# bjg-gh/style_transfer_visualizer

Hardware: AMD Instinct MI355X
Metric: optimization steps/sec at 512² and 1024², 1/2/4/8 MI355X (higher is better)
Workload: dtype bf16; 1 GPU; single 512x512 image per GPU, L-BFGS (max_iter=1, history 100), VGG19 bf16 storage / fp32 accumulate, fp32 Gram, --no-video (BASELINE.json configs[1]); weights: synthetic He-scaled; size=512, images=1, init_method=random, parallelism=replicas x1 (independent images), lbfgs_history_prefill_steps=95, world_size=1

## Files before the change

include/stv.h:

```cpp
#ifndef STV_H_
#define STV_H_

#include <stddef.h>
#include <stdint.h>

#ifdef __cplusplus
extern "C" {
#endif

enum { STV_F32 = 0, STV_BF16 = 1, STV_BF16X3 = 2 };

enum {
  STV_OK = 0,
  STV_ERR_ARG = 1,
  STV_ERR_LAUNCH = 2,
  STV_ERR_ALLOC = 3,
  STV_ERR_GRAPH = 4
};

enum {
  STV_RELU_IN = 1,
  STV_RELU_OUT = 2,
  STV_MASK = 4,
  STV_ACCUM = 8,
// ... 140 lines not shown
#define STV_GIF_THREADS 256
#define STV_GIF_MAX_BLOCKS 2048
#define STV_GIF_HIST_BINS 32768
int stv_frame_hist(const uint8_t* frame_hwc, size_t n_pixels, uint32_t* hist, void* stream);
int stv_gif_map(const uint8_t* frame_hwc, uint8_t* index_hw, int H, int W, const uint8_t* palette, int n_colors, int spread,
                void* stream);

#define STV_JPEG_DCT_TABLE                                        \
  {{2896, 2896, 2896, 2896, 2896, 2896, 2896, 2896},              \
   {4017, 3406, 2276, 799, -799, -2276, -3406, -4017},            \
   {3784, 1567, -1567, -3784, -3784, -1567, 1567, 3784},          \
   {3406, -799, -4017, -2276, 2276, 4017, 799, -3406},            \
   {2896, -2896, -2896, 2896, 2896, -2896, -2896, 2896},          \
   {2276, -4017, 799, 3406, -3406, -799, 4017, -2276},            \
   {1567, -3784, 3784, -1567, -1567, 3784, -3784, 1567},          \
   {799, -2276, 3406, -4017, 4017, -3406, 2276, -799}}
#define STV_JPEG_DCT_THREADS 256
#define STV_JPEG_THREADS 256
#define STV_JPEG_MAX_BLOCK_BITS 1664
#define STV_JPEG_MAX_DIM 65535
int stv_jpeg_dct(const uint8_t* frame_hwc, const int* qtabs, int H, int W, int16_t* coef, void* stream);
int stv_jpeg_block_bits(const int16_t* coef, int n_frames, int blocks_per_frame, uint32_t* bits, void* stream);
int stv_jpeg_scan(const uint32_t* bits, int n_frames, int blocks_per_frame, uint32_t* offsets, uint32_t* totals, void* stream);
int stv_jpeg_emit(const int16_t* coef, const uint32_t* offsets, const uint32_t* base, int n_frames, int blocks_per_frame,
                  uint8_t* stream_bytes, size_t capacity, void* stream);

int stv_loss_combine(const float* parts, const int32_t* table, const float* scale,
                     int n_terms, float style_w, float content_w, float* losses,
                     float* scores, void* stream);
int stv_loss_combine_log(const float* parts, const int32_t* table, const float* scale,
                         int n_terms, float style_w, float content_w, float* losses,
                         float* scores, float* log_ring, int log_capacity, uint32_t* log_count,
                         uint32_t* log_seq, void* stream);
int stv_host_mailbox_alloc(size_t bytes, void** out);
void stv_host_mailbox_free(void* p);


typedef struct stv_lbfgs_state stv_lbfgs_state;
size_t stv_lbfgs_state_bytes(int history);
size_t stv_lbfgs_workspace_bytes(size_t n, int history);
int stv_lbfgs_step(float* x, const float* grad, void* state, void* workspace, size_t n,
                   int history, int m_max, float lr, float tol_grad, float tol_change,
                   void* stream);
size_t stv_lbfgsc_state_bytes(int history);
size_t stv_lbfgsc_workspace_bytes(size_t n, int history);
int stv_lbfgsc_step(float* x, const float* grad, void* state, void* workspace, size_t n,
                    int history, int m_max, float lr, float tol_grad, float tol_change,
                    void* stream);
int stv_lbfgsc_dots(const float* grad, void* state, void* workspace, size_t n, int history, int m_max, void* stream);
int stv_lbfgsc_apply(float* x, const float* grad, void* state, void* workspace, size_t n, int history, float lr,
                     float tol_grad, float tol_change, void* stream);
size_t stv_lbfgsc_dots_offset(size_t n, int history, int* count, int* max_index);
int stv_lbfgsc_geometry(size_t n, int history, size_t* nn, int* tile_a, int* ntiles, int* pgroups, int* tile_b);
int stv_lbfgsc_iter(float* x, const float* grad, const float* loss, void* state, void* workspace, size_t n,
                    int history, int m_max, int iters_per_step, float lr, float tol_grad, float tol_change,
                    void* stream);
int stv_lbfgsc_iter_reset(void* state, void* stream);
int stv_adam_step(float* x, const float* grad, float* exp_avg, float* exp_avg_sq, size_t n,
                  float lr, float one_minus_beta1, float beta2, float one_minus_beta2, float eps,
                  float bias_c1, float bias_c2_sqrt, void* stream);

enum {
  STV_OP_CONV_FIRST_FWD = 1, STV_OP_CONV_FIRST_DGRAD, STV_OP_CONV, STV_OP_POOL_FWD,
  STV_OP_POOL_BWD, STV_OP_RELU_FWD, STV_OP_RELU_BWD, STV_OP_GRAM_PARTIAL,
  STV_OP_GRAM_FINISH, STV_OP_CONTENT_LOSS, STV_OP_CONTENT_GRAD, STV_OP_LOSS_COMBINE,
  STV_OP_MEMSET, STV_OP_GRAM_MULTI, STV_OP_LBFGS_STEP, STV_OP_LBFGS_ITER, STV_OP_TV,
  STV_OP_LAP, STV_OP_MASK_SPLIT, STV_OP_AVGPOOL_FWD, STV_OP_AVGPOOL_BWD
};
typedef struct {
  int32_t op, dtype, flags, taps;
  int32_t H, W, cin, cout;
  int64_t n;
  float f0, f1, f2, f3;
  const void* p0; const void* p1; const void* p2; const void* p3;
  void* q0; void* q1; void* q2; void* q3;
} stv_op_t;

typedef struct stv_program stv_program;
int stv_program_create(const stv_op_t* ops, int n_ops, stv_program** out);
int stv_program_run(stv_program* prog, int use_graph, void* stream);
int stv_program_profile(stv_program* prog, void* stream, float* ms_out, int n_out);
int stv_program_profile_reps(stv_program* prog, void* stream, int reps, float* ms_out, int n_out);
int stv_program_op_count(const stv_program* prog);
void stv_program_destroy(stv_program* prog);

#ifdef __cplusplus
}
#endif
#endif
```

style_transfer_visualizer_amd/_lib.py:

```python
from __future__ import annotations

import ctypes
import os
from ctypes import c_float, c_int, c_int32, c_int64, c_size_t, c_void_p

_HERE = os.path.dirname(os.path.abspath(__file__))
LIB_PATH = os.environ.get("STV_LIB_PATH") or os.path.join(_HERE, "libstv_hip.so")

STV_F32, STV_BF16, STV_BF16X3 = 0, 1, 2
TUNE_BF16X3 = 6
RELU_IN, RELU_OUT, MASK, ACCUM, W_BLOCKED, POOL_IDX, POOL_ROUTE, POOL_ONLY = 1, 2, 4, 8, 16, 32, 64, 128

(OP_CONV_FIRST_FWD, OP_CONV_FIRST_DGRAD, OP_CONV, OP_POOL_FWD, OP_POOL_BWD, OP_RELU_FWD,
 OP_RELU_BWD, OP_GRAM_PARTIAL, OP_GRAM_FINISH, OP_CONTENT_LOSS, OP_CONTENT_GRAD,
 OP_LOSS_COMBINE, OP_MEMSET, OP_GRAM_MULTI, OP_LBFGS_STEP, OP_LBFGS_ITER, OP_TV, OP_LAP, OP_MASK_SPLIT, OP_AVGPOOL_FWD, OP_AVGPOOL_BWD) = range(1, 22)

CONTENT_LOSS_PARTS = 256
TV_LOSS_PARTS = 256
TV_THREADS, TV_VEC = 1024, 4
KIND_STYLE, KIND_CONTENT, KIND_EXTRA = 0, 1, 2
LAP_POOL, LAP_LOSS, LAP_GRAD = 0, 1, 2
LAP_POOLS = (1, 2, 4, 8, 16, 32)
LAP_THREADS, LAP_TILE_H, LAP_TILE_W, LAP_LOSS_PARTS, LAP_GRAD_MAX_BLOCKS, LAP_VEC = 256, 8, 32, 256, 512, 4
MASK_MAX_REGIONS, MASK_SPLIT_THREADS, MASK_SPLIT_MAX_BLOCKS = 4, 256, 1024
# ... 70 lines not shown
    "stv_conv_tune": (c_int, [c_int, c_int, c_int, c_int, c_int, c_int, c_void_p]),
    "stv_conv_tune_export": (c_int, [ctypes.POINTER(c_int), c_int]),
    "stv_conv_tune_import": (c_int, [ctypes.POINTER(c_int), c_int]),
    "stv_conv_next_weights": (None, [c_void_p, c_size_t]),
    "stv_conv_num_configs": (c_int, []),
    "stv_conv_last_launch": (c_int, []),
    "stv_conv_uses_ws": (c_int, [c_int, c_int, c_int, c_int, c_int, c_int, c_int, c_int, c_int]),
    "stv_conv_config": (c_int, [c_int, c_int, c_int, c_int, c_int, c_int]),
    "stv_maxpool_fwd": (c_int, [c_void_p, c_void_p, c_int, c_int, c_int, c_int, c_void_p]),
    "stv_maxpool_bwd": (c_int, [c_void_p, c_void_p, c_void_p, c_int, c_int, c_int, c_int, c_int, c_void_p]),
    "stv_avgpool_fwd": (c_int, [c_void_p, c_void_p, c_int, c_int, c_int, c_int, c_int, c_void_p]),
    "stv_avgpool_bwd": (c_int, [c_void_p, c_void_p, c_void_p, c_int, c_int, c_int, c_int, c_int, c_void_p]),
    "stv_relu_fwd": (c_int, [c_void_p, c_void_p, c_size_t, c_int, c_void_p]),
    "stv_relu_bwd": (c_int, [c_void_p, c_void_p, c_void_p, c_size_t, c_int, c_int, c_void_p]),
    "stv_gram_partial": (c_int, [c_void_p, c_void_p, c_int, c_int, c_int, c_void_p]),
    "stv_gram_finish": (c_int, [c_void_p, c_void_p, c_void_p, c_void_p, c_void_p, c_int, c_int, c_float, c_float, c_float, c_void_p, c_int, c_void_p]),
    "stv_gram_multi": (c_int, [c_void_p, c_int, c_int, c_void_p]),
    "stv_content_loss": (c_int, [c_void_p, c_void_p, c_void_p, c_size_t, c_int, c_void_p]),
    "stv_content_loss_grad": (c_int, [c_void_p, c_void_p, c_void_p, c_void_p, c_size_t, c_float, c_int, c_void_p]),
    "stv_content_grad": (c_int, [c_void_p, c_void_p, c_void_p, c_size_t, c_float, c_void_p, c_int, c_int, c_void_p]),
    "stv_tv": (c_int, [c_void_p, c_void_p, c_void_p, c_int, c_int, c_int, c_float, c_int, c_void_p]),
    "stv_lap": (c_int, [c_void_p, c_void_p, c_void_p, c_void_p, c_void_p, c_int, c_int, c_int, c_int, c_float, c_int, c_int, c_void_p]),
    "stv_mask_split": (c_int, [c_void_p, c_void_p, c_void_p, c_size_t, c_int, c_int, c_int, c_void_p]),
    "stv_resize2x": (c_int, [c_void_p, c_void_p, c_int, c_int, c_int, c_int, c_void_p]),
    "stv_resize_axis": (c_int, [c_void_p, c_void_p, c_int, c_int, c_int, c_int, c_int, c_void_p, c_void_p, c_void_p, c_int, c_void_p]),
    "stv_color_stats": (c_int, [c_void_p, c_void_p, c_int, c_int, c_void_p]),
    "stv_color_affine": (c_int, [c_void_p, c_void_p, ctypes.POINTER(c_float), c_int, c_int, c_void_p]),
    "stv_luma_transfer": (c_int, [c_void_p, c_void_p, c_void_p, c_int, c_int, ctypes.POINTER(c_float), ctypes.POINTER(c_float), c_void_p]),
    "stv_kmeans_assign": (c_int, [c_void_p, c_void_p, c_void_p, c_void_p, c_int, c_int, c_int, c_void_p]),
    "stv_gram_blend": (c_int, [c_void_p, c_void_p, ctypes.POINTER(c_float), c_int, c_int64, c_void_p]),
    "stv_image_to_u8": (c_int, [c_void_p, c_void_p, c_int, c_int, ctypes.POINTER(c_float), ctypes.POINTER(c_float), c_int, c_void_p]),
    "stv_frame_hist": (c_int, [c_void_p, c_size_t, c_void_p, c_void_p]),
    "stv_gif_map": (c_int, [c_void_p, c_void_p, c_int, c_int, c_void_p, c_int, c_int, c_void_p]),
    "stv_jpeg_dct": (c_int, [c_void_p, ctypes.POINTER(c_int), c_int, c_int, c_void_p, c_void_p]),
    "stv_jpeg_block_bits": (c_int, [c_void_p, c_int, c_int, c_void_p, c_void_p]),
    "stv_jpeg_scan": (c_int, [c_void_p, c_int, c_int, c_void_p, c_void_p, c_void_p]),
    "stv_jpeg_emit": (c_int, [c_void_p, c_void_p, c_void_p, c_int, c_int, c_void_p, c_size_t, c_void_p]),
    "stv_loss_combine": (c_int, [c_void_p, c_void_p, c_void_p, c_int, c_float, c_float, c_void_p, c_void_p, c_void_p]),
    "stv_loss_combine_log": (c_int, [c_void_p, c_void_p, c_void_p, c_int, c_float, c_float, c_void_p, c_void_p, c_void_p,
                                     c_int, c_void_p, c_void_p, c_void_p]),
    "stv_host_mailbox_alloc": (c_int, [c_size_t, ctypes.POINTER(c_void_p)]),
    "stv_host_mailbox_free": (None, [c_void_p]),
    "stv_lbfgs_state_bytes": (c_size_t, [c_int]),
    "stv_lbfgs_workspace_bytes": (c_size_t, [c_size_t, c_int]),
    "stv_lbfgs_step": (c_int, [c_void_p, c_void_p, c_void_p, c_void_p, c_size_t, c_int, c_int, c_float, c_float, c_float, c_void_p]),
    "stv_lbfgsc_state_bytes": (c_size_t, [c_int]),
    "stv_lbfgsc_workspace_bytes": (c_size_t, [c_size_t, c_int]),
    "stv_lbfgsc_step": (c_int, [c_void_p, c_void_p, c_void_p, c_void_p, c_size_t, c_int, c_int, c_float, c_float, c_float, c_void_p]),
    "stv_lbfgsc_dots": (c_int, [c_void_p, c_void_p, c_void_p, c_size_t, c_int, c_int, c_void_p]),
    "stv_lbfgsc_apply": (c_int, [c_void_p, c_void_p, c_void_p, c_void_p, c_size_t, c_int, c_float, c_float, c_float, c_void_p]),
    "stv_lbfgsc_dots_offset": (c_size_t, [c_size_t, c_int, ctypes.POINTER(c_int), ctypes.POINTER(c_int)]),
    "stv_lbfgsc_geometry": (c_int, [c_size_t, c_int, ctypes.POINTER(c_size_t), ctypes.POINTER(c_int), ctypes.POINTER(c_int),
                                    ctypes.POINTER(c_int), ctypes.POINTER(c_int)]),
    "stv_lbfgsc_iter": (c_int, [c_void_p, c_void_p, c_void_p, c_void_p, c_void_p, c_size_t, c_int, c_int, c_int, c_float, c_float, c_float,
                                c_void_p]),
    "stv_lbfgsc_iter_reset": (c_int, [c_void_p, c_void_p]),
    "stv_adam_step": (c_int, [c_void_p, c_void_p, c_void_p, c_void_p, c_size_t, c_float, c_float, c_float, c_float, c_float, c_float, c_float, c_void_p]),
    "stv_program_create": (c_int, [ctypes.POINTER(StvOp), c_int, ctypes.POINTER(c_void_p)]),
    "stv_program_run": (c_int, [c_void_p, c_int, c_void_p]),
    "stv_program_profile": (c_int, [c_void_p, c_void_p, ctypes.POINTER(c_float), c_int]),
    "stv_program_profile_reps": (c_int, [c_void_p, c_void_p, c_int, ctypes.POINTER(c_float), c_int]),
    "stv_program_op_count": (c_int, [c_void_p]),
    "stv_program_destroy": (None, [c_void_p]),
}

_lib = None


def load() -> ctypes.CDLL:
    global _lib
    if _lib is not None:
        return _lib
    import torch
    if not os.path.exists(LIB_PATH):
        msg = (f"{LIB_PATH} not found: build it with `python -c 'import __graft_entry__ as g; g.build()'` "
               "(hipcc --offload-arch=gfx950). There is no CPU/eager fallback for this path.")
        raise RuntimeError(msg)
    lib = ctypes.CDLL(LIB_PATH)
    for name, (res, args) in SIGNATURES.items():
        fn = getattr(lib, name)
        fn.restype = res
        fn.argtypes = args
    _lib = lib
    _import_tile_table(lib)
    return lib


TILE_TABLE_PATH = os.environ.get("STV_TILE_TABLE") or os.path.join(_HERE, "conv_tiles_gfx950.json")
tile_table_info: dict = {"source": None, "entries": 0}


def _import_tile_table(lib: ctypes.CDLL) -> None:
    import json
    import warnings
    if not os.path.exists(TILE_TABLE_PATH):
        return

    def give_up(why: str) -> None:
        lib.stv_conv_tune_import(None, 0)
        tile_table_info.update(source=None, entries=0, ignored=f"{os.path.basename(TILE_TABLE_PATH)}: {why}")
        warnings.warn(f"conv tile table {TILE_TABLE_PATH} ignored ({why}): analytic tile choices", RuntimeWarning, stacklevel=3)
    try:
        with open(TILE_TABLE_PATH) as fh:
            doc = json.load(fh)
        rows = [int(v) for e in doc.get("entries", []) for v in (e["H"], e["W"], e["cin"], e["cout"], e["taps"], e["elem_bytes"], e["cfg"])]
    except (OSError, ValueError, KeyError, TypeError, AttributeError) as exc:
# ... 42 lines not shown
```

style_transfer_visualizer_amd/csrc/lbfgs_compact.hip:

```cpp
#include <stddef.h>
#include <stdlib.h>

#include <type_traits>

#include "stv_common.h"

namespace {

constexpr int MAX_HIST = 128;
constexpr int MAX_S = MAX_HIST + 1;
constexpr int NSCAL = 8;
constexpr int SC_DTMAX = 7;

struct CState {
  int n_iter, hist_len, head, skip, no_update, pushed, steps_seen, step_pos;
  float t, H_diag, gtd, gmax, ys, yy, cg, prev_loss;
  float ro[MAX_S];
  float cs[MAX_S];
  float cy[MAX_S];
};

struct CWs {
  float* d;
  float* prev_g;
// ... 97 lines not shown
  const int per = (m + pgroups - 1) / pgroups;
  const int j_end = (pgrp + 1) * per < m ? (pgrp + 1) * per : m;
  for (int jj = pgrp * per; jj < j_end; ++jj) {
    const int slot = (head + jj) % S;
    const float* __restrict__ sj = w.S + (size_t)slot * nn;
    const float* __restrict__ yj = w.Y + (size_t)slot * nn;
    double a0 = 0.0, a1 = 0.0, a2 = 0.0, a4 = 0.0;
#pragma unroll
    for (int u = 0; u < U; ++u) {
      const size_t idx = base + (size_t)(u * 256 + tid) * 4;
      const f32x4 s4 = ldh4(sj + idx);
      const f32x4 y4 = ldh4(yj + idx);
#pragma unroll
      for (int e = 0; e < 4; ++e) {
        const double sd = (double)s4[e], yd = (double)y4[e];
        const double gd = (double)gv[u][e], cd = (double)yv[u][e];
        a0 = fma(sd, gd, a0);
        a1 = fma(yd, gd, a1);
        a2 = fma(sd, cd, a2);
        a4 = fma(yd, cd, a4);
      }
    }
    a0 = wave_sum_d_dpp(a0); a1 = wave_sum_d_dpp(a1); a2 = wave_sum_d_dpp(a2); a4 = wave_sum_d_dpp(a4);
    if (lane == 0) {
      double* o = w.part + (size_t)(jj * 5) * nparts + p;
      o[0] = a0; o[(size_t)nparts] = a1; o[(size_t)2 * nparts] = a2; o[(size_t)3 * nparts] = 0.0;
      o[(size_t)4 * nparts] = a4;
    }
  }
  if (pgrp != 0) return;
  gmax = wave_max(gmax);
  gl1 = wave_sum_d(gl1); gg = wave_sum_d(gg); gs = wave_sum_d(gs); gy = wave_sum_d(gy); sy = wave_sum_d(sy); yy = wave_sum_d(yy);
  if (lane == 0) {
    double* o = w.partd + p;
    o[0] = (double)gmax; o[(size_t)nparts] = gl1; o[(size_t)2 * nparts] = gg; o[(size_t)3 * nparts] = gs;
    o[(size_t)4 * nparts] = gy; o[(size_t)5 * nparts] = sy; o[(size_t)6 * nparts] = yy;
  }
  if constexpr (ITER) {
    dtmax = wave_max(dtmax);
    if (lane == 0) w.partd[(size_t)SC_DTMAX * nparts + p] = (double)dtmax;
  }
}
template <int U>
__global__ __launch_bounds__(256) void pass_a_kernel(const float* __restrict__ g, const CState* st, CWs w,
                                                     size_t n, size_t nn, int hist, int nparts, int ntiles, int pgroups) {
  pass_a_body<U, false>(g, st, w, n, nn, hist, nparts, ntiles, pgroups);
}
template <int U>
__global__ __launch_bounds__(256) void pass_a_iter_kernel(const float* __restrict__ g, const CState* st, CWs w,
                                                          size_t n, size_t nn, int hist, int nparts, int ntiles, int pgroups) {
  pass_a_body<U, true>(g, st, w, n, nn, hist, nparts, ntiles, pgroups);
}

__global__ __launch_bounds__(256) void reduce_kernel(const CState* st, CWs w, int hist, int nparts) {
  __shared__ double red[256];
  const int m = st->hist_len;
  int dot = blockIdx.x;
  const bool scalar = dot >= 5 * m;
  if (scalar) dot = 5 * hist + (dot - 5 * m);
  if (dot >= 5 * hist + NSCAL) return;
  const double* __restrict__ src = w.part + (size_t)dot * nparts;
  const double* __restrict__ srcd = w.partd + (size_t)(scalar ? dot - 5 * hist : 0) * nparts;
  const bool is_max = dot == 5 * hist || dot == 5 * hist + SC_DTMAX;
  double acc = 0.0;
  for (int i = threadIdx.x; i < nparts; i += 256) {
    const double v = scalar ? srcd[i] : src[i];
    acc = is_max ? fmax(acc, v) : acc + v;
  }
  red[threadIdx.x] = acc;
  __syncthreads();
  for (int s = 128; s > 0; s >>= 1) {
    if (threadIdx.x < s)
      red[threadIdx.x] = is_max ? fmax(red[threadIdx.x], red[threadIdx.x + s]) : red[threadIdx.x] + red[threadIdx.x + s];
    __syncthreads();
  }
  if (threadIdx.x == 0) w.dots[scalar ? 5 * MAX_HIST + (dot - 5 * hist) : dot] = red[0];
}

#ifdef STV_SOLVE_STAMPS
__device__ unsigned long long g_solve_stamps[8];
#define SOLVE_STAMP(k) do { if (threadIdx.x == 0) g_solve_stamps[k] = wall_clock64(); } while (0)
#else
#define SOLVE_STAMP(k) do { } while (0)
#endif

template <bool ITER>
__device__ __forceinline__ void solve_body(CState* st, CWs w, int hist, float lr, float tol_grad, float tol_change,
                                           const float* __restrict__ loss, int iters) {
  extern __shared__ __attribute__((aligned(16))) char smem_raw[];
  const int S = hist + 1;
  const int P = hist | 1;
  double* sT = reinterpret_cast<double*>(smem_raw);
  __shared__ int sh_skip, sh_pushed, sh_m, sh_head, sh_cslot, sh_mold, sh_pos;
  __shared__ float sh_newro, sh_H;
  __shared__ double sh_gs[MAX_S], sh_gy[MAX_S], sh_ro[MAX_S];
  __shared__ double sh_bp[2][128];
  __shared__ double sh_cy[128];
  const int tid = threadIdx.x;
  const double* D = w.dots;
  const double* SC = w.dots + 5 * MAX_HIST;
  const double gmax = SC[0], gl1 = SC[1], gg = SC[2], gsc = SC[3], gyc = SC[4], ys = SC[5], yy = SC[6];
  SOLVE_STAMP(0);

  if (tid == 0) {
    struct Hdr { int n_iter, hist_len, head, skip, no_update, pushed, steps_seen, step_pos;
                 float t, H_diag, gtd, gmax, ys, yy, cg, prev_loss; };
    static_assert(sizeof(Hdr) == 64, "header layout");
    Hdr h = *reinterpret_cast<const Hdr*>(st);
    h.steps_seen += 1;
    h.gmax = (float)gmax;
    h.no_update = 0;
    h.pushed = 0;
    int skip = ((float)gmax <= tol_grad) ? 1 : 0;
    int pos = 1;
    float loss_now = 0.f;
    if constexpr (ITER) {
      loss_now = *loss;
      int done = h.step_pos < 0 ? -h.step_pos : h.step_pos;
      bool dead = h.step_pos < 0;
      if (done >= iters) { done = 0; dead = false; }
      pos = done + 1;
      if (pos > 1 && !skip)
        skip = ((float)SC[SC_DTMAX] <= tol_change || fabs((double)loss_now - (double)h.prev_loss) < (double)tol_change) ? 1 : 0;
      if (dead) skip = 1;
      h.step_pos = pos >= iters ? 0 : (skip ? -pos : pos);
    }
    h.skip = skip;
    int pushed = 0;
    const int m_old = h.hist_len;
    const int cslot = (h.head + m_old) % S;
    if (!skip) {
      h.n_iter += 1;
      if (h.n_iter == 1) {
        h.hist_len = 0;
        h.head = 0;
        h.H_diag = 1.0f;
      } else {
        h.ys = (float)ys;
        h.yy = (float)yy;
        if ((float)ys > 1e-10f) {
          pushed = 1;
          if (h.hist_len == hist) h.head = (h.head + 1) % S;
          else h.hist_len += 1;
          st->ro[cslot] = 1.0f / (float)ys;
          h.H_diag = (float)ys / (float)yy;
          sh_newro = 1.0f / (float)ys;
        }
      }
      if (h.n_iter == 1) {
// ... 26 lines not shown
      w.YY[(size_t)slot * S + cslot] = y_j_yc;
      w.YY[(size_t)cslot * S + slot] = y_j_yc;
    }
    if (tid == 0) {
      w.SY[(size_t)cslot * S + cslot] = ys;
      w.YY[(size_t)cslot * S + cslot] = yy;
    }
  }
  for (int i = tid; i < m; i += 256) {
    const int slot = (head + i) % S;
    sh_ro[i] = (sh_pushed && slot == cslot) ? (double)sh_newro : (double)st->ro[slot];
    if (sh_pushed && slot == cslot) {
      sh_gs[i] = gsc;
      sh_gy[i] = gyc;
    } else {
      const int jj = (slot - old_head + S) % S;
      sh_gs[i] = D[jj * 5 + 0];
      sh_gy[i] = D[jj * 5 + 1];
    }
  }
  __threadfence_block();
  __syncthreads();
  SOLVE_STAMP(2);
  {
    const int j = tid & 127, i0 = tid >> 7;
    if (j < m) {
      int col = head + j;
      if (col >= S) col -= S;
      constexpr int FB = 50;
      for (int ib = i0; ib < m; ib += 2 * FB) {
        double v[FB];
#pragma unroll
        for (int k = 0; k < FB; ++k) {
          int i = ib + 2 * k;
          if (i >= m) i = m - 1;
          int rs = head + i;
          if (rs >= S) rs -= S;
          const double* __restrict__ src = (i < j) ? w.SY : w.YY;
          v[k] = src[(size_t)rs * S + col];
        }
#pragma unroll
        for (int k = 0; k < FB; ++k) {
          const int i = ib + 2 * k;
          if (i < m) sT[i * P + j] = v[k];
        }
      }
    }
  }
  __syncthreads();
  SOLVE_STAMP(3);

  const int lane = tid & 63, wave4 = tid >> 6;
  const int j0 = lane, j1 = lane + 64;
  auto bcast = [](double v, int src) -> double {
    const long long bits = __double_as_longlong(v);
    const int lo = __builtin_amdgcn_readlane((int)(bits & 0xFFFFFFFFll), src);
    const int hi = __builtin_amdgcn_readlane((int)(bits >> 32), src);
    return __longlong_as_double(((long long)hi << 32) | (unsigned int)lo);
  };
  const double gs0 = j0 < m ? sh_gs[j0] : 0.0, gs1 = j1 < m ? sh_gs[j1] : 0.0;
  const double gy0 = j0 < m ? sh_gy[j0] : 0.0, gy1 = j1 < m ? sh_gy[j1] : 0.0;
  const double ro0 = j0 < m ? sh_ro[j0] : 0.0, ro1 = j1 < m ? sh_ro[j1] : 0.0;
  double cy0 = 0.0, cy1 = 0.0, cs0 = 0.0, cs1 = 0.0, al0 = 0.0, al1 = 0.0;
  double a0 = 0.0, a1 = 0.0;
  double cg = -1.0;
  constexpr int CH = 4;
  using hi_t = std::integral_constant<bool, true>;
  using lo_t = std::integral_constant<bool, false>;
  const int r0 = (j0 < m ? j0 : m - 1) * P, r1 = (j1 < m ? j1 : m - 1) * P;
  const int q0 = j0 < m ? j0 : m - 1, q1 = j1 < m ? j1 : m - 1;
  const float ro0f = (float)ro0, ro1f = (float)ro1;
  auto walk1 = [&](auto HI, int ifrom, int ito) {
    constexpr bool hi = decltype(HI)::value;
    if (ifrom < ito) return;
    double n0[CH], n1[CH];
    auto fetch = [&](int ib) {
#pragma unroll
      for (int k = 0; k < CH; ++k) {
        const int i = max(ib - k, 0);
        const double v0 = sT[r0 + i];
        if (hi) {
          n0[k] = v0;
          const double v1 = sT[r1 + i];
          n1[k] = (j1 < i) ? v1 : 0.0;
        } else {
          n0[k] = (j0 < i) ? v0 : 0.0;
        }
      }
    };
    fetch(ifrom);
    for (int ib = ifrom; ib >= ito; ib -= CH) {
      double c0[CH], c1[CH];
#pragma unroll
      for (int k = 0; k < CH; ++k) { c0[k] = n0[k]; c1[k] = hi ? n1[k] : 0.0; }
      if (ib - CH >= ito) fetch(ib - CH);
#pragma unroll
      for (int k = 0; k < CH; ++k) {
        const int i = ib - k;
        if (i < ito) break;
        const int src = hi ? i - 64 : i;
        const double cand = (double)(float)((float)(cg * (hi ? gs1 : gs0) + (hi ? a1 : a0)) * (hi ? ro1f : ro0f));
        const double al = bcast(cand, src);
        if (lane == src) {
          if (hi) { al1 = al; cy1 = -al; } else { al0 = al; cy0 = -al; }
        }
        a0 -= al * c0[k];
        if (hi) a1 -= al * c1[k];
      }
    }
  };
  if (m > 0) {
    walk1(hi_t{}, m - 1, 64);
    walk1(lo_t{}, m - 1 < 63 ? m - 1 : 63, 0);
  }
  SOLVE_STAMP(4);
  const double H = (double)sh_H;
  cg *= H; cy0 *= H; cy1 *= H;
  double b0 = cg * gy0, b1 = cg * gy1;
  {
    if (wave4 == 0) {
      sh_cy[j0] = cy0;
      sh_cy[j1] = cy1;
    }
    __syncthreads();
    const int row = tid & 127, part = tid >> 7;
    double chunk_sum[2] = {0.0, 0.0};
    if (row < m) {
      const int rb = row * P;
#pragma unroll
      for (int c = 0; c < 2; ++c) {
        const int jb = (2 * part + c) * 32;
        double acc = 0.0;
#pragma unroll
        for (int kb = 0; kb < 32; kb += 16) {
          double cv[16], tv[16];
#pragma unroll
          for (int k = 0; k < 16; ++k) {
            const int j = jb + kb + k;
            const int jc = j < m ? j : m - 1;
            cv[k] = sh_cy[j];
            tv[k] = sT[(jc <= row) ? rb + jc : jc * P + row];
          }
#pragma unroll
          for (int k = 0; k < 16; ++k) acc = fma(cv[k], tv[k], acc);
        }
        chunk_sum[c] = acc;
      }
    }
    sh_bp[part][row] = chunk_sum[0] + chunk_sum[1];
    __syncthreads();
    if (tid >= 64) return;
    b0 = b0 + (sh_bp[0][lane] + sh_bp[1][lane]);
    b1 = b1 + (sh_bp[0][64 + lane] + sh_bp[1][64 + lane]);
  }
  SOLVE_STAMP(5);
  auto walk3 = [&](auto HI, int ifrom, int ito) {
    constexpr bool hi = decltype(HI)::value;
    if (ifrom >= ito) return;
    double n0[CH], n1[CH];
    auto fetch = [&](int ib) {
#pragma unroll
      for (int k = 0; k < CH; ++k) {
        const int i = min(ib + k, m - 1);
        const double v1 = sT[i * P + q1];
        if (!hi) {
          const double v0 = sT[i * P + q0];
          n0[k] = (j0 > i) ? v0 : 0.0;
          n1[k] = v1;
        } else {
          n1[k] = (j1 > i) ? v1 : 0.0;
        }
      }
    };
    fetch(ifrom);
    for (int ib = ifrom; ib < ito; ib += CH) {
      double c0[CH], c1[CH];
#pragma unroll
      for (int k = 0; k < CH; ++k) { c0[k] = hi ? 0.0 : n0[k]; c1[k] = n1[k]; }
      if (ib + CH < ito) fetch(ib + CH);
#pragma unroll
      for (int k = 0; k < CH; ++k) {
        const int i = ib + k;
        if (i >= ito) break;
        const int src = hi ? i - 64 : i;
        const double be = (double)(float)((float)(hi ? b1 : b0) * (hi ? ro1f : ro0f));
        const double cand = (double)(float)((float)(hi ? al1 : al0) - (float)be);
        const double csi = bcast(cand, src);
        if (lane == src) {
          if (hi) cs1 = csi; else cs0 = csi;
        }
        if (!hi) b0 += csi * c0[k];
        b1 += csi * c1[k];
      }
    }
  };
  walk3(lo_t{}, 0, m < 64 ? m : 64);
  walk3(hi_t{}, 64, m);
  SOLVE_STAMP(6);
  double gtd = 0.0;
  if (j0 < m) gtd += cy0 * sh_gy[j0] + cs0 * sh_gs[j0];
  if (j1 < m) gtd += cy1 * sh_gy[j1] + cs1 * sh_gs[j1];
  gtd = wave_sum_d(gtd) + cg * gg;
  if (j0 < m) { st->cs[(head + j0) % S] = (float)cs0; st->cy[(head + j0) % S] = (float)cy0; }
  if (j1 < m) { st->cs[(head + j1) % S] = (float)cs1; st->cy[(head + j1) % S] = (float)cy1; }
  if (lane == 0) {
    st->cg = (float)cg;
    st->gtd = (float)gtd;
    const int no_update = ((float)gtd > -tol_change) ? 1 : 0;
    st->no_update = no_update;
    if constexpr (ITER)
      if (no_update && sh_pos < iters) st->step_pos = -sh_pos;
  }
  SOLVE_STAMP(7);
}
__global__ __launch_bounds__(256) void solve_kernel(CState* st, CWs w, int hist, float lr, float tol_grad,
                                                    float tol_change) {
  solve_body<false>(st, w, hist, lr, tol_grad, tol_change, nullptr, 1);
}
__global__ __launch_bounds__(256) void solve_iter_kernel(CState* st, CWs w, int hist, float lr, float tol_grad,
                                                         float tol_change, const float* __restrict__ loss, int iters) {
  solve_body<true>(st, w, hist, lr, tol_grad, tol_change, loss, iters);
}

template <int U>
__global__ __launch_bounds__(256) void pass_b_kernel(float* __restrict__ x, const float* __restrict__ g,
                                                     const CState* st, CWs w, size_t n, size_t nn, int hist) {
  if (st->skip) return;
  const int S = hist + 1;
  const int tid = threadIdx.x;
  const size_t base = (size_t)blockIdx.x * (256 * 4 * U);
  const int m = st->hist_len, head = st->head;
  const float cg = st->cg, t = st->t;
  const bool move = st->no_update == 0;
  double acc[U][4];
  f32x4 gv[U];
#pragma unroll
  for (int u = 0; u < U; ++u) {
    const size_t idx = base + (size_t)(u * 256 + tid) * 4;
    gv[u] = ld4_guard(g, idx, n);
#pragma unroll
    for (int e = 0; e < 4; ++e) acc[u][e] = (double)cg * (double)gv[u][e];
  }
  for (int jj = m - 1; jj >= 0; --jj) {
    const int slot = (head + jj) % S;
    const double cs = (double)st->cs[slot], cy = (double)st->cy[slot];
    const float* __restrict__ sj = w.S + (size_t)slot * nn;
    const float* __restrict__ yj = w.Y + (size_t)slot * nn;
#pragma unroll
    for (int u = 0; u < U; ++u) {
      const size_t idx = base + (size_t)(u * 256 + tid) * 4;
      const f32x4 s4 = ldh4(sj + idx);
// ... 66 lines not shown

template <typename K>
inline K by_tile(int tile, K k1, K k2, K k4) { return tile == 4096 ? k4 : tile == 2048 ? k2 : k1; }

int launch_dots(const float* grad, void* state, void* workspace, size_t n, int history, int m_max, void* stream,
                bool iter) {
  if (!grad || !state || !workspace || n == 0) return STV_ERR_ARG;
  if (history < 1 || history > MAX_HIST) return STV_ERR_ARG;
  if (m_max < 0) m_max = 0;
  if (m_max > history) m_max = history;
  hipStream_t st = static_cast<hipStream_t>(stream);
  CState* s = static_cast<CState*>(state);
  const StepGeom g = step_geom(workspace, n, history);
  const auto sweep_a = iter ? by_tile(g.tile, pass_a_iter_kernel<1>, pass_a_iter_kernel<2>, pass_a_iter_kernel<4>)
                            : by_tile(g.tile, pass_a_kernel<1>, pass_a_kernel<2>, pass_a_kernel<4>);
  hipLaunchKernelGGL(sweep_a, dim3(g.ntiles * g.pgroups), dim3(256), 0, st, grad, s, g.w, n, g.nn, history, g.nparts, g.ntiles,
                     g.pgroups);
  hipLaunchKernelGGL(reduce_kernel, dim3(5 * m_max + NSCAL), dim3(256), 0, st, s, g.w, history, g.nparts);
  STV_CHECK_LAUNCH();
  return STV_OK;
}

int launch_apply(float* x, const float* grad, const float* loss, void* state, void* workspace, size_t n, int history,
                 int iters, float lr, float tol_grad, float tol_change, void* stream) {
  if (!x || !grad || !state || !workspace || n == 0) return STV_ERR_ARG;
  if (history < 1 || history > MAX_HIST) return STV_ERR_ARG;
  hipStream_t st = static_cast<hipStream_t>(stream);
  CState* s = static_cast<CState*>(state);
  const StepGeom g = step_geom(workspace, n, history);
  const size_t lds = (size_t)history * (size_t)(history | 1) * sizeof(double);
  const void* solve_fn = loss ? reinterpret_cast<const void*>(&solve_iter_kernel) : reinterpret_cast<const void*>(&solve_kernel);
  if (stv_set_max_lds(solve_fn, MAX_HIST * (MAX_HIST | 1) * (int)sizeof(double)) != STV_OK)
    return STV_ERR_LAUNCH;
  if (loss) hipLaunchKernelGGL(solve_iter_kernel, dim3(1), dim3(256), lds, st, s, g.w, history, lr, tol_grad, tol_change, loss, iters);
  else hipLaunchKernelGGL(solve_kernel, dim3(1), dim3(256), lds, st, s, g.w, history, lr, tol_grad, tol_change);
  const int tile_b = tile_floats_b(n);
  hipLaunchKernelGGL(by_tile(tile_b, pass_b_kernel<1>, pass_b_kernel<2>, pass_b_kernel<4>), dim3((int)(g.nn / tile_b)), dim3(256),
                     0, st, x, grad, s, g.w, n, g.nn, history);
  STV_CHECK_LAUNCH();
  return STV_OK;
}
}

extern "C" int stv_lbfgsc_dots(const float* grad, void* state, void* workspace, size_t n, int history, int m_max,
                               void* stream) {
  return launch_dots(grad, state, workspace, n, history, m_max, stream, false);
}

extern "C" int stv_lbfgsc_apply(float* x, const float* grad, void* state, void* workspace, size_t n, int history,
                                float lr, float tol_grad, float tol_change, void* stream) {
  return launch_apply(x, grad, nullptr, state, workspace, n, history, 1, lr, tol_grad, tol_change, stream);
}

extern "C" size_t stv_lbfgsc_dots_offset(size_t n, int history, int* count, int* max_index) {
  const size_t nn = align_up(n, 4096);
  const int S = history + 1;
  if (count) *count = 5 * MAX_HIST + NSCAL;
  if (max_index) *max_index = 5 * MAX_HIST;
  return (nn * (2 + 2 * (size_t)S) + 2 * 2 * align_up((size_t)S * S, 64)) * sizeof(float);
}

extern "C" int stv_lbfgsc_geometry(size_t n, int history, size_t* nn, int* tile_a, int* ntiles, int* pgroups, int* tile_b) {
  if (n == 0 || history < 1 || history > MAX_HIST) return STV_ERR_ARG;
  const StepGeom g = launch_geom(n);
  if (nn) *nn = g.nn;
  if (tile_a) *tile_a = g.tile;
  if (ntiles) *ntiles = g.ntiles;
  if (pgroups) *pgroups = g.pgroups;
  if (tile_b) *tile_b = tile_floats_b(n);
  return STV_OK;
}

extern "C" int stv_lbfgsc_step(float* x, const float* grad, void* state, void* workspace, size_t n, int history,
                               int m_max, float lr, float tol_grad, float tol_change, void* stream) {
  if (!x) return STV_ERR_ARG;
  const int rc = stv_lbfgsc_dots(grad, state, workspace, n, history, m_max, stream);
  if (rc != STV_OK) return rc;
  return stv_lbfgsc_apply(x, grad, state, workspace, n, history, lr, tol_grad, tol_change, stream);
}

extern "C" int stv_lbfgsc_iter(float* x, const float* grad, const float* loss, void* state, void* workspace, size_t n,
                               int history, int m_max, int iters_per_step, float lr, float tol_grad, float tol_change,
                               void* stream) {
  if (!x || !loss || iters_per_step < 1 || iters_per_step > 32767) return STV_ERR_ARG;
  const int rc = launch_dots(grad, state, workspace, n, history, m_max, stream, true);
  if (rc != STV_OK) return rc;
  return launch_apply(x, grad, loss, state, workspace, n, history, iters_per_step, lr, tol_grad, tol_change, stream);
}

extern "C" int stv_lbfgsc_iter_reset(void* state, void* stream) {
  if (!state) return STV_ERR_ARG;
  if (hipMemsetAsync(static_cast<char*>(state) + offsetof(CState, step_pos), 0, sizeof(int), static_cast<hipStream_t>(stream)) != hipSuccess)
    return STV_ERR_LAUNCH;
  return STV_OK;
}

#ifdef STV_SOLVE_STAMPS
extern "C" int stv_debug_solve_stamps(unsigned long long* out8) {
  return hipMemcpyFromSymbol(out8, HIP_SYMBOL(g_solve_stamps), sizeof(g_solve_stamps)) == hipSuccess ? 0 : 1;
}
#endif
```

style_transfer_visualizer_amd/csrc/program.hip:

```cpp
#include <stdlib.h>

#include <vector>

#include "stv_common.h"

struct stv_program {
  std::vector<stv_op_t> ops;
  hipGraph_t graph = nullptr;
  hipGraphExec_t exec = nullptr;
  hipStream_t captured_on = nullptr;
  std::vector<std::vector<stv_gram_tap_t>> tap_tables;
};

namespace {

int run_op(const stv_op_t& o, void* st) {
  switch (o.op) {
    case STV_OP_CONV_FIRST_FWD:
      return stv_conv_first_fwd(static_cast<const float*>(o.p0), static_cast<const float*>(o.p3),
                                static_cast<const float*>(o.p2), o.q0, static_cast<float*>(o.q1), o.H, o.W, o.cin,
                                o.cout, o.dtype, st);
    case STV_OP_CONV_FIRST_DGRAD:
      return stv_conv_first_dgrad(o.p0, static_cast<const float*>(o.p2), static_cast<float*>(o.q0), o.H,
                                  o.W, o.cin, o.cout, o.dtype, st);
// ... 38 lines not shown
                                  static_cast<const float*>(o.p2), o.cin, o.f0, o.f1,
                                  static_cast<float*>(o.q0), static_cast<float*>(o.q1), static_cast<float*>(o.q2),
                                  (int)o.n, static_cast<uint32_t*>(o.q3), static_cast<uint32_t*>(const_cast<void*>(o.p3)), st);
    case STV_OP_GRAM_MULTI:
      return stv_gram_multi(static_cast<const stv_gram_tap_t*>(o.p0), (int)o.n, o.dtype, st);
    case STV_OP_LBFGS_STEP:
      return stv_lbfgsc_step(static_cast<float*>(o.q0), static_cast<const float*>(o.p0), o.q1, o.q2, (size_t)o.n, o.cin, o.cout,
                             o.f0, o.f1, o.f2, st);
    case STV_OP_LBFGS_ITER:
      return stv_lbfgsc_iter(static_cast<float*>(o.q0), static_cast<const float*>(o.p0), static_cast<const float*>(o.p1), o.q1, o.q2,
                             (size_t)o.n, o.cin, o.cout, o.taps, o.f0, o.f1, o.f2, st);
    case STV_OP_TV:
      return stv_tv(static_cast<const float*>(o.p0), static_cast<float*>(o.q0), static_cast<float*>(o.q1), o.cin, o.H, o.W,
                    o.f0, o.flags, st);
    case STV_OP_LAP:
      return stv_lap(static_cast<const float*>(o.p0), static_cast<const float*>(o.p1), static_cast<float*>(o.q0),
                     static_cast<float*>(o.q1), static_cast<float*>(o.q2), o.cin, o.H, o.W, o.cout, o.f0, o.taps, o.flags, st);
    case STV_OP_MASK_SPLIT:
      return stv_mask_split(o.p0, static_cast<const uint8_t*>(o.p1), o.q0, (size_t)o.n, o.cin, o.cout, o.dtype, st);
    case STV_OP_MEMSET:
      if (hipMemsetAsync(o.q0, 0, (size_t)o.n, static_cast<hipStream_t>(st)) != hipSuccess)
        return STV_ERR_LAUNCH;
      return STV_OK;
    default:
      return STV_ERR_ARG;
  }
}

void hint_next_weights(const std::vector<stv_op_t>& ops, size_t i) {
  static const bool on = !(getenv("STV_NEXT_W") && atoi(getenv("STV_NEXT_W")) == 0);
  if (!on || ops[i].op != STV_OP_CONV) return;
  for (size_t j = i + 1; j < ops.size(); ++j) {
    const stv_op_t& nx = ops[j];
    if (nx.op == STV_OP_CONV && nx.taps == 9) {
      stv_conv_next_weights(nx.p1, (size_t)9 * nx.cin * nx.cout * (nx.dtype == STV_BF16 ? 2 : 4));
      return;
    }
  }
}

int run_all(stv_program* p, void* st) {
  const size_t n_ops = p->ops.size();
  for (size_t i = 0; i < n_ops; ++i) {
    hint_next_weights(p->ops, i);
    const int rc = run_op(p->ops[i], st);
    stv_conv_next_weights(nullptr, 0);
    if (rc != STV_OK) return rc;
  }
  return STV_OK;
}

}

extern "C" int stv_version(void) { return 117; }

extern "C" int stv_program_create(const stv_op_t* ops, int n_ops, stv_program** out) {
  if (!ops || n_ops <= 0 || !out) return STV_ERR_ARG;
  stv_program* p = new (std::nothrow) stv_program();
  if (!p) return STV_ERR_ALLOC;
  p->ops.assign(ops, ops + n_ops);
  for (stv_op_t& o : p->ops) {
    if (o.op != STV_OP_GRAM_MULTI) continue;
    if (!o.p0 || o.n <= 0 || o.n > 8) {
      delete p;
      return STV_ERR_ARG;
    }
    const stv_gram_tap_t* src = static_cast<const stv_gram_tap_t*>(o.p0);
    p->tap_tables.emplace_back(src, src + o.n);
  }
  size_t k = 0;
  for (stv_op_t& o : p->ops)
    if (o.op == STV_OP_GRAM_MULTI) o.p0 = p->tap_tables[k++].data();
  *out = p;
  return STV_OK;
}

extern "C" int stv_program_run(stv_program* prog, int use_graph, void* stream) {
  if (!prog) return STV_ERR_ARG;
  hipStream_t st = static_cast<hipStream_t>(stream);
  if (!use_graph || st == nullptr) return run_all(prog, stream);
  if (prog->exec && prog->captured_on != st) {
    (void)hipGraphExecDestroy(prog->exec);
    (void)hipGraphDestroy(prog->graph);
    prog->exec = nullptr;
    prog->graph = nullptr;
  }
  if (!prog->exec) {
    int rc = run_all(prog, stream);
    if (rc != STV_OK) return rc;
    if (hipStreamBeginCapture(st, hipStreamCaptureModeThreadLocal) != hipSuccess) {
      (void)hipGetLastError();
      return STV_ERR_GRAPH;
    }
    rc = run_all(prog, stream);
    hipGraph_t g = nullptr;
    if (hipStreamEndCapture(st, &g) != hipSuccess || rc != STV_OK) {
      if (g) (void)hipGraphDestroy(g);
      (void)hipGetLastError();
      return rc != STV_OK ? rc : STV_ERR_GRAPH;
    }
    hipGraphExec_t e = nullptr;
    if (hipGraphInstantiate(&e, g, nullptr, nullptr, 0) != hipSuccess) {
      (void)hipGraphDestroy(g);
      (void)hipGetLastError();
      return STV_ERR_GRAPH;
    }
    prog->graph = g;
// ... 48 lines not shown
```

style_transfer_visualizer_amd/ops.py:

```python
from __future__ import annotations

import ctypes
import functools

import numpy as np
import torch

from . import _lib
from . import resize as _resize
from ._lib import ACCUM, MASK, POOL_ONLY, RELU_IN, RELU_OUT, STV_BF16, STV_BF16X3, STV_F32, W_BLOCKED


def dtype_code(dtype: torch.dtype, *, split: bool = False) -> int:
    if split:
        if dtype != torch.float32:
            msg = f"split-bf16 products (bf16x3) need fp32 storage, got {dtype}"
            raise RuntimeError(msg)
        return STV_BF16X3
    if dtype == torch.float32:
        return STV_F32
    if dtype == torch.bfloat16:
        return STV_BF16
    msg = f"unsupported activation dtype {dtype}; use torch.float32 or torch.bfloat16"
    raise RuntimeError(msg)
# ... 770 lines not shown
    work = torch.zeros((ws_bytes + 3) // 4, dtype=torch.float32, device=device)
    return state, work


def lbfgs_step(x: torch.Tensor, grad: torch.Tensor, state: torch.Tensor, work: torch.Tensor, history: int,
               m_max: int, lr: float, tol_grad: float = 1e-7, tol_change: float = 1e-9, *,
               compact: bool = False) -> None:
    lib = _lib.load()
    fn = lib.stv_lbfgsc_step if compact else lib.stv_lbfgs_step
    _lib.check(fn(_ptr(x), _ptr(grad), _ptr(state), _ptr(work), x.numel(), history, m_max, lr,
                  tol_grad, tol_change, _stream()), "stv_lbfgsc_step" if compact else "stv_lbfgs_step")


def lbfgs_iter(x: torch.Tensor, grad: torch.Tensor, loss: torch.Tensor, state: torch.Tensor, work: torch.Tensor,
               history: int, m_max: int, iters_per_step: int, lr: float, tol_grad: float = 1e-7,
               tol_change: float = 1e-9) -> None:
    if not loss.is_cuda or loss.dtype != torch.float32 or loss.numel() != 1:
        msg = "lbfgs_iter needs the loss as a one-element float32 GPU tensor"
        raise RuntimeError(msg)
    lib = _lib.load()
    _lib.check(lib.stv_lbfgsc_iter(_ptr(x), _ptr(grad), _ptr(loss), _ptr(state), _ptr(work), x.numel(), history, m_max,
                                   iters_per_step, lr, tol_grad, tol_change, _stream()), "stv_lbfgsc_iter")


def lbfgs_iter_reset(state: torch.Tensor) -> None:
    _lib.check(_lib.load().stv_lbfgsc_iter_reset(_ptr(state), _stream()), "stv_lbfgsc_iter_reset")


def lbfgs_dots(grad: torch.Tensor, state: torch.Tensor, work: torch.Tensor, history: int, m_max: int) -> torch.Tensor:
    lib = _lib.load()
    n = grad.numel()
    _lib.check(lib.stv_lbfgsc_dots(_ptr(grad), _ptr(state), _ptr(work), n, history, m_max, _stream()), "stv_lbfgsc_dots")
    return lbfgs_dots_view(work, n, history)[0]


def lbfgs_dots_view(work: torch.Tensor, n: int, history: int) -> tuple[torch.Tensor, int]:
    count, imax = ctypes.c_int(), ctypes.c_int()
    off = int(_lib.load().stv_lbfgsc_dots_offset(n, history, ctypes.byref(count), ctypes.byref(imax)))
    if off % 8:
        msg = "internal: unaligned inner-product block"
        raise RuntimeError(msg)
    return work[off // 4: off // 4 + 2 * count.value].view(torch.float64), imax.value


def lbfgs_geometry(n: int, history: int) -> dict:
    nn = ctypes.c_size_t()
    tile_a, ntiles, pgroups, tile_b = ctypes.c_int(), ctypes.c_int(), ctypes.c_int(), ctypes.c_int()
    _lib.check(_lib.load().stv_lbfgsc_geometry(n, history, ctypes.byref(nn), ctypes.byref(tile_a), ctypes.byref(ntiles),
                                               ctypes.byref(pgroups), ctypes.byref(tile_b)), "stv_lbfgsc_geometry")
    return {"nn": int(nn.value), "tile_a": tile_a.value, "ntiles": ntiles.value, "pgroups": pgroups.value,
            "tile_b": tile_b.value}


def lbfgs_views(work: torch.Tensor, n: int, history: int) -> dict:
    nn = lbfgs_geometry(n, history)["nn"]
    rows = history + 1
    ring = work[2 * nn: 2 * nn + 2 * rows * nn].view(2, rows, nn)
    return {"d": work[:nn], "prev_g": work[nn: 2 * nn], "S": ring[0], "Y": ring[1]}


def lbfgs_apply(x: torch.Tensor, grad: torch.Tensor, state: torch.Tensor, work: torch.Tensor, history: int, lr: float,
                tol_grad: float = 1e-7, tol_change: float = 1e-9) -> None:
    lib = _lib.load()
    _lib.check(lib.stv_lbfgsc_apply(_ptr(x), _ptr(grad), _ptr(state), _ptr(work), x.numel(), history, lr, tol_grad,
                                    tol_change, _stream()), "stv_lbfgsc_apply")


def adam_step(x: torch.Tensor, grad: torch.Tensor, exp_avg: torch.Tensor, exp_avg_sq: torch.Tensor, step: int,
              lr: float = 1e-3, betas: tuple[float, float] = (0.9, 0.999), eps: float = 1e-8) -> None:
    b1, b2 = betas
    bc1 = 1 - b1 ** step
    bc2_sqrt = (1 - b2 ** step) ** 0.5
    lib = _lib.load()
    _lib.check(lib.stv_adam_step(_ptr(x), _ptr(grad), _ptr(exp_avg), _ptr(exp_avg_sq), x.numel(), lr, 1 - b1, b2,
                                 1 - b2, eps, bc1, bc2_sqrt, _stream()), "stv_adam_step")
```

Measured before the change: 1156 steps/s.

## Speed up L-BFGS dot reductions and overlap two-loop recursion with row sums

Rewrites the L-BFGS partial-sum reduce kernel to use 16-way unrolled loads and wavefront DPP/shuffle reductions in place of a shared-memory tree with many barriers. It skips one of the five dot families (index 3) by writing zero. In the solve kernel, the first recursion walk is split into four 32-row chunks so other waves compute the matrix-row products for finished chunks while wave 0 continues. Broadcasts now use single fp32 readlanes instead of paired 32-bit readlanes of doubles. A standalone reduce entry point and a Python wrapper are also added. This adds complexity, and correctness depends on the skipped dot really being unused.

```diff
diff --git a/include/stv.h b/include/stv.h
--- a/include/stv.h
+++ b/include/stv.h
@@ -216,6 +216,8 @@
                      float tol_grad, float tol_change, void* stream);
 size_t stv_lbfgsc_dots_offset(size_t n, int history, int* count, int* max_index);
 int stv_lbfgsc_geometry(size_t n, int history, size_t* nn, int* tile_a, int* ntiles, int* pgroups, int* tile_b);
+int stv_lbfgsc_reduce(const void* state, const double* part, const double* partd, double* dots, int history, int nparts,
+                      int m_max, void* stream);
 int stv_lbfgsc_iter(float* x, const float* grad, const float* loss, void* state, void* workspace, size_t n,
                     int history, int m_max, int iters_per_step, float lr, float tol_grad, float tol_change,
                     void* stream);
diff --git a/style_transfer_visualizer_amd/_lib.py b/style_transfer_visualizer_amd/_lib.py
--- a/style_transfer_visualizer_amd/_lib.py
+++ b/style_transfer_visualizer_amd/_lib.py
@@ -146,6 +146,7 @@
     "stv_lbfgsc_dots_offset": (c_size_t, [c_size_t, c_int, ctypes.POINTER(c_int), ctypes.POINTER(c_int)]),
     "stv_lbfgsc_geometry": (c_int, [c_size_t, c_int, ctypes.POINTER(c_size_t), ctypes.POINTER(c_int), ctypes.POINTER(c_int),
                                     ctypes.POINTER(c_int), ctypes.POINTER(c_int)]),
+    "stv_lbfgsc_reduce": (c_int, [c_void_p, c_void_p, c_void_p, c_void_p, c_int, c_int, c_int, c_void_p]),
     "stv_lbfgsc_iter": (c_int, [c_void_p, c_void_p, c_void_p, c_void_p, c_void_p, c_size_t, c_int, c_int, c_int, c_float, c_float, c_float,
                                 c_void_p]),
     "stv_lbfgsc_iter_reset": (c_int, [c_void_p, c_void_p]),
diff --git a/style_transfer_visualizer_amd/csrc/lbfgs_compact.hip b/style_transfer_visualizer_amd/csrc/lbfgs_compact.hip
--- a/style_transfer_visualizer_amd/csrc/lbfgs_compact.hip
+++ b/style_transfer_visualizer_amd/csrc/lbfgs_compact.hip
@@ -173,29 +173,59 @@
   pass_a_body<U, true>(g, st, w, n, nn, hist, nparts, ntiles, pgroups);
 }
 
+template <int N>
+__device__ __forceinline__ double row_down_d(double v) {
+  const long long b = __double_as_longlong(v);
+  const int lo = __builtin_amdgcn_update_dpp(0, (int)(b & 0xFFFFFFFFll), 0x100 + N, 0xF, 0xF, false);
+  const int hi = __builtin_amdgcn_update_dpp(0, (int)(b >> 32), 0x100 + N, 0xF, 0xF, false);
+  return __longlong_as_double(((long long)hi << 32) | (unsigned int)lo);
+}
+
+template <bool MAX>
+__device__ __forceinline__ void reduce_body(const double* __restrict__ p, int nparts, double* red, double* out) {
+  auto op = [](double a, double b) { return MAX ? fmax(a, b) : a + b; };
+  constexpr int RB = 16;
+  const int tid = threadIdx.x;
+  double acc = 0.0;
+  for (int i0 = tid; i0 < nparts; i0 += 256 * RB) {
+    double v[RB];
+#pragma unroll
+    for (int k = 0; k < RB; ++k) {
+      const int i = i0 + 256 * k;
+      v[k] = p[i < nparts ? i : nparts - 1];
+    }
+#pragma unroll
+    for (int k = 0; k < RB; ++k)
+      if (i0 + 256 * k < nparts) acc = op(acc, v[k]);
+  }
+  red[tid] = acc;
+  __syncthreads();
+  if (tid < 64) {
+    double v = op(op(red[tid], red[tid + 128]), op(red[tid + 64], red[tid + 192]));
+    v = op(v, __shfl_down(v, 32, 64));
+    v = op(v, __shfl_down(v, 16, 64));
+    v = op(v, row_down_d<8>(v));
+    v = op(v, row_down_d<4>(v));
+    v = op(v, row_down_d<2>(v));
+    v = op(v, row_down_d<1>(v));
+    if (tid == 0) *out = v;
+  }
+}
 __global__ __launch_bounds__(256) void reduce_kernel(const CState* st, CWs w, int hist, int nparts) {
   __shared__ double red[256];
   const int m = st->hist_len;
   int dot = blockIdx.x;
   const bool scalar = dot >= 5 * m;
   if (scalar) dot = 5 * hist + (dot - 5 * m);
-  if (dot >= 5 * hist + NSCAL) return;
-  const double* __restrict__ src = w.part + (size_t)dot * nparts;
-  const double* __restrict__ srcd = w.partd + (size_t)(scalar ? dot - 5 * hist : 0) * nparts;
-  const bool is_max = dot == 5 * hist || dot == 5 * hist + SC_DTMAX;
-  double acc = 0.0;
-  for (int i = threadIdx.x; i < nparts; i += 256) {
-    const double v = scalar ? srcd[i] : src[i];
-    acc = is_max ? fmax(acc, v) : acc + v;
-  }
-  red[threadIdx.x] = acc;
-  __syncthreads();
-  for (int s = 128; s > 0; s >>= 1) {
-    if (threadIdx.x < s)
-      red[threadIdx.x] = is_max ? fmax(red[threadIdx.x], red[threadIdx.x + s]) : red[threadIdx.x] + red[threadIdx.x + s];
-    __syncthreads();
-  }
-  if (threadIdx.x == 0) w.dots[scalar ? 5 * MAX_HIST + (dot - 5 * hist) : dot] = red[0];
+  if (dot >= 5 * hist + NSCAL || (!scalar && dot % 5 == 3)) {
+    if (dot < 5 * hist && threadIdx.x == 0) w.dots[dot] = 0.0;
+    return;
+  }
+  const double* __restrict__ p = scalar ? w.partd + (size_t)(dot - 5 * hist) * nparts
+                                        : w.part + (size_t)dot * nparts;
+  double* out = w.dots + (scalar ? 5 * MAX_HIST + (dot - 5 * hist) : dot);
+  if (dot == 5 * hist || dot == 5 * hist + SC_DTMAX) reduce_body<true>(p, nparts, red, out);
+  else reduce_body<false>(p, nparts, red, out);
 }
 
 #ifdef STV_SOLVE_STAMPS
@@ -215,7 +245,7 @@
   __shared__ int sh_skip, sh_pushed, sh_m, sh_head, sh_cslot, sh_mold, sh_pos;
   __shared__ float sh_newro, sh_H;
   __shared__ double sh_gs[MAX_S], sh_gy[MAX_S], sh_ro[MAX_S];
-  __shared__ double sh_bp[2][128];
+  __shared__ double sh_cs[4][128];
   __shared__ double sh_cy[128];
   const int tid = threadIdx.x;
   const double* D = w.dots;
@@ -348,16 +378,15 @@
 
   const int lane = tid & 63, wave4 = tid >> 6;
   const int j0 = lane, j1 = lane + 64;
-  auto bcast = [](double v, int src) -> double {
-    const long long bits = __double_as_longlong(v);
-    const int lo = __builtin_amdgcn_readlane((int)(bits & 0xFFFFFFFFll), src);
-    const int hi = __builtin_amdgcn_readlane((int)(bits >> 32), src);
-    return __longlong_as_double(((long long)hi << 32) | (unsigned int)lo);
+  auto bcast_f = [](float v, int src) -> float {
+    return __builtin_bit_cast(float, __builtin_amdgcn_readlane(__builtin_bit_cast(int, v), src));
   };
+  auto keep_f = [lane](float v, int src, float own) -> float { return lane == src ? v : own; };
   const double gs0 = j0 < m ? sh_gs[j0] : 0.0, gs1 = j1 < m ? sh_gs[j1] : 0.0;
   const double gy0 = j0 < m ? sh_gy[j0] : 0.0, gy1 = j1 < m ? sh_gy[j1] : 0.0;
   const double ro0 = j0 < m ? sh_ro[j0] : 0.0, ro1 = j1 < m ? sh_ro[j1] : 0.0;
-  double cy0 = 0.0, cy1 = 0.0, cs0 = 0.0, cs1 = 0.0, al0 = 0.0, al1 = 0.0;
+  float al0f = 0.f, al1f = 0.f, cs0f = 0.f, cs1f = 0.f;
+  auto cy_of = [m](float alf, int j) { return j < m ? -(double)alf : 0.0; };
   double a0 = 0.0, a1 = 0.0;
   double cg = -1.0;
   constexpr int CH = 4;
@@ -395,60 +424,55 @@
         const int i = ib - k;
         if (i < ito) break;
         const int src = hi ? i - 64 : i;
-        const double cand = (double)(float)((float)(cg * (hi ? gs1 : gs0) + (hi ? a1 : a0)) * (hi ? ro1f : ro0f));
-        const double al = bcast(cand, src);
-        if (lane == src) {
-          if (hi) { al1 = al; cy1 = -al; } else { al0 = al; cy0 = -al; }
-        }
+        const float cand = (float)(cg * (hi ? gs1 : gs0) + (hi ? a1 : a0)) * (hi ? ro1f : ro0f);
+        const float alf = bcast_f(cand, src);
+        if (hi) al1f = keep_f(alf, src, al1f); else al0f = keep_f(alf, src, al0f);
+        const double al = (double)alf;
         a0 -= al * c0[k];
         if (hi) a1 -= al * c1[k];
       }
     }
   };
-  if (m > 0) {
-    walk1(hi_t{}, m - 1, 64);
-    walk1(lo_t{}, m - 1 < 63 ? m - 1 : 63, 0);
+  const double H = (double)sh_H;
+  auto chunk_rows = [&](int c, int row) {
+    double acc = 0.0;
+    if (row < m) {
+      const int rb = row * P, jb = c * 32;
+#pragma unroll
+      for (int kb = 0; kb < 32; kb += 16) {
+        double cv[16], tv[16];
+#pragma unroll
+        for (int k = 0; k < 16; ++k) {
+          const int j = jb + kb + k;
+          const int jc = j < m ? j : m - 1;
+          cv[k] = sh_cy[j];
+          tv[k] = sT[(jc <= row) ? rb + jc : jc * P + row];
+        }
+#pragma unroll
+        for (int k = 0; k < 16; ++k) acc = fma(cv[k], tv[k], acc);
+      }
+    }
+    sh_cs[c][row] = acc;
+  };
+  for (int c = 3; c >= 0; --c) {
+    if (wave4 == 0) {
+      const int ifrom = m - 1 < 32 * c + 31 ? m - 1 : 32 * c + 31;
+      if (c >= 2) walk1(hi_t{}, ifrom, 32 * c); else walk1(lo_t{}, ifrom, 32 * c);
+      if ((lane >> 5) == (c & 1)) sh_cy[32 * c + (lane & 31)] = (c >= 2 ? cy_of(al1f, j1) : cy_of(al0f, j0)) * H;
+    } else if (wave4 <= 2 && c < 3) {
+      chunk_rows(c + 1, tid - 64);
+    }
+    __syncthreads();
   }
   SOLVE_STAMP(4);
-  const double H = (double)sh_H;
-  cg *= H; cy0 *= H; cy1 *= H;
+  if (tid < 128) chunk_rows(0, tid);
+  __syncthreads();
+  if (tid >= 64) return;
+  cg *= H;
+  const double cy0 = cy_of(al0f, j0) * H, cy1 = cy_of(al1f, j1) * H;
   double b0 = cg * gy0, b1 = cg * gy1;
-  {
-    if (wave4 == 0) {
-      sh_cy[j0] = cy0;
-      sh_cy[j1] = cy1;
-    }
-    __syncthreads();
-    const int row = tid & 127, part = tid >> 7;
-    double chunk_sum[2] = {0.0, 0.0};
-    if (row < m) {
-      const int rb = row * P;
-#pragma unroll
-      for (int c = 0; c < 2; ++c) {
-        const int jb = (2 * part + c) * 32;
-        double acc = 0.0;
-#pragma unroll
-        for (int kb = 0; kb < 32; kb += 16) {
-          double cv[16], tv[16];
-#pragma unroll
-          for (int k = 0; k < 16; ++k) {
-            const int j = jb + kb + k;
-            const int jc = j < m ? j : m - 1;
-            cv[k] = sh_cy[j];
-            tv[k] = sT[(jc <= row) ? rb + jc : jc * P + row];
-          }
-#pragma unroll
-          for (int k = 0; k < 16; ++k) acc = fma(cv[k], tv[k], acc);
-        }
-        chunk_sum[c] = acc;
-      }
-    }
-    sh_bp[part][row] = chunk_sum[0] + chunk_sum[1];
-    __syncthreads();
-    if (tid >= 64) return;
-    b0 = b0 + (sh_bp[0][lane] + sh_bp[1][lane]);
-    b1 = b1 + (sh_bp[0][64 + lane] + sh_bp[1][64 + lane]);
-  }
+  b0 = b0 + ((sh_cs[0][lane] + sh_cs[1][lane]) + (sh_cs[2][lane] + sh_cs[3][lane]));
+  b1 = b1 + ((sh_cs[0][64 + lane] + sh_cs[1][64 + lane]) + (sh_cs[2][64 + lane] + sh_cs[3][64 + lane]));
   SOLVE_STAMP(5);
   auto walk3 = [&](auto HI, int ifrom, int ito) {
     constexpr bool hi = decltype(HI)::value;
@@ -479,12 +503,9 @@
         const int i = ib + k;
         if (i >= ito) break;
         const int src = hi ? i - 64 : i;
-        const double be = (double)(float)((float)(hi ? b1 : b0) * (hi ? ro1f : ro0f));
-        const double cand = (double)(float)((float)(hi ? al1 : al0) - (float)be);
-        const double csi = bcast(cand, src);
-        if (lane == src) {
-          if (hi) cs1 = csi; else cs0 = csi;
-        }
+        const float csf = bcast_f(__builtin_fmaf(-(hi ? ro1f : ro0f), (float)(hi ? b1 : b0), hi ? al1f : al0f), src);
+        if (hi) cs1f = keep_f(csf, src, cs1f); else cs0f = keep_f(csf, src, cs0f);
+        const double csi = (double)csf;
         if (!hi) b0 += csi * c0[k];
         b1 += csi * c1[k];
       }
@@ -493,6 +514,7 @@
   walk3(lo_t{}, 0, m < 64 ? m : 64);
   walk3(hi_t{}, 64, m);
   SOLVE_STAMP(6);
+  const double cs0 = (double)cs0f, cs1 = (double)cs1f;
   double gtd = 0.0;
   if (j0 < m) gtd += cy0 * sh_gy[j0] + cs0 * sh_gs[j0];
   if (j1 < m) gtd += cy1 * sh_gy[j1] + cs1 * sh_gs[j1];
@@ -665,6 +687,22 @@
   return launch_apply(x, grad, nullptr, state, workspace, n, history, 1, lr, tol_grad, tol_change, stream);
 }
 
+extern "C" int stv_lbfgsc_reduce(const void* state, const double* part, const double* partd, double* dots, int history,
+                                 int nparts, int m_max, void* stream) {
+  if (!state || !part || !partd || !dots || nparts < 1) return STV_ERR_ARG;
+  if (history < 1 || history > MAX_HIST) return STV_ERR_ARG;
+  if (m_max < 0) m_max = 0;
+  if (m_max > history) m_max = history;
+  CWs w{};
+  w.part = const_cast<double*>(part);
+  w.partd = const_cast<double*>(partd);
+  w.dots = dots;
+  hipLaunchKernelGGL(reduce_kernel, dim3(5 * m_max + NSCAL), dim3(256), 0, static_cast<hipStream_t>(stream),
+                     static_cast<const CState*>(state), w, history, nparts);
+  STV_CHECK_LAUNCH();
+  return STV_OK;
+}
+
 extern "C" size_t stv_lbfgsc_dots_offset(size_t n, int history, int* count, int* max_index) {
   const size_t nn = align_up(n, 4096);
   const int S = history + 1;
diff --git a/style_transfer_visualizer_amd/csrc/program.hip b/style_transfer_visualizer_amd/csrc/program.hip
--- a/style_transfer_visualizer_amd/csrc/program.hip
+++ b/style_transfer_visualizer_amd/csrc/program.hip
@@ -114,7 +114,7 @@
 
 }
 
-extern "C" int stv_version(void) { return 117; }
+extern "C" int stv_version(void) { return 118; }
 
 extern "C" int stv_program_create(const stv_op_t* ops, int n_ops, stv_program** out) {
   if (!ops || n_ops <= 0 || !out) return STV_ERR_ARG;
diff --git a/style_transfer_visualizer_amd/ops.py b/style_transfer_visualizer_amd/ops.py
--- a/style_transfer_visualizer_amd/ops.py
+++ b/style_transfer_visualizer_amd/ops.py
@@ -846,6 +846,20 @@
             "tile_b": tile_b.value}
 
 
+def lbfgs_reduce(state: torch.Tensor, part: torch.Tensor, partd: torch.Tensor, dots: torch.Tensor, history: int,
+                 m_max: int) -> None:
+    if part.dtype != torch.float64 or partd.dtype != torch.float64 or dots.dtype != torch.float64:
+        msg = "lbfgs_reduce works on float64 partial sums"
+        raise RuntimeError(msg)
+    nparts = partd.shape[1]
+    if part.shape != (5 * history, nparts) or partd.shape[0] != 8 or dots.numel() < 5 * 128 + 8 or not (
+            part.is_contiguous() and partd.is_contiguous() and dots.is_contiguous()):
+        msg = f"lbfgs_reduce: part {tuple(part.shape)}, partd {tuple(partd.shape)}, dots {dots.numel()} do not fit history {history}"
+        raise RuntimeError(msg)
+    _lib.check(_lib.load().stv_lbfgsc_reduce(_ptr(state), _ptr(part), _ptr(partd), _ptr(dots), history, nparts, m_max,
+                                             _stream()), "stv_lbfgsc_reduce")
+
+
 def lbfgs_views(work: torch.Tensor, n: int, history: int) -> dict:
     nn = lbfgs_geometry(n, history)["nn"]
     rows = history + 1
```

Measured after the change: 1159 steps/s, median of 4. Within noise of the previous version (+0.3%).
